# nirvanesque/headCT_foundation

Hardware: AMD Instinct MI355X
Metric: CT-volumes/sec MAE pretrain step (96^3, ViT-B/16^3, mask 0.75) (higher is better)
Workload: dtype bf16; 1 GPU; BASELINE config #2: MAE ViT-B/16^3, 96^3x1ch, mask 0.75, full train step (fwd+bwd+clip+AdamW+LR); per_gpu_batch=256, global_batch=256, parallelism=dp1, init=reference init, seed 42

## Files before the change

### headct_foundation_amd/_lib.py

```python
from __future__ import annotations

import ctypes as C
import os
from typing import Optional

HERE = os.path.dirname(os.path.abspath(__file__))
LIB_PATH = os.path.join(HERE, "libheadct_hip.so")

HCT_F32, HCT_BF16, HCT_F16 = 0, 1, 2
NORM_LAYERNORM, NORM_RMSNORM = 0, 1
HCT_ACT_NONE, HCT_ACT_GELU, HCT_ACT_DGELU, HCT_ACT_TANH, HCT_ACT_GELU_D, HCT_ACT_MULAUX = 0, 1, 2, 3, 4, 5
ACT_NONE, ACT_GELU, ACT_DGELU = 0, 1, 2

c_void_p, c_int, c_float, c_size_t, c_int64 = C.c_void_p, C.c_int, C.c_float, C.c_size_t, C.c_int64


class GemmArgs(C.Structure):
    _fields_ = [
        ("M", c_int), ("N", c_int), ("K", c_int),
        ("A", c_void_p), ("a_dtype", c_int), ("lda", c_int64), ("transA", c_int),
        ("B", c_void_p), ("b_dtype", c_int), ("ldb", c_int64), ("transB", c_int),
        ("C", c_void_p), ("c_dtype", c_int), ("ldc", c_int64),
        ("bias", c_void_p), ("residual", c_void_p), ("ldr", c_int64),
        ("act", c_int),
# ... 51 lines not shown
    "hct_assemble_bwd_workspace_bytes": (c_size_t, [c_int]),
    "hct_layernorm_fwd": (c_int, [c_void_p, c_void_p, c_void_p, c_int, c_int, c_float, c_void_p, c_int, c_void_p, c_void_p, c_void_p]),
    "hct_layernorm_bwd_workspace_bytes": (c_size_t, [c_int, c_int]),
    "hct_layernorm_bwd": (c_int, [c_void_p, c_int, c_void_p, c_void_p, c_void_p, c_void_p, c_void_p, c_int, c_int, c_void_p, c_void_p,
                                  c_int, c_void_p, c_void_p, c_void_p, c_void_p, c_size_t, c_void_p]),
    "hct_layernorm_bwd_mapped": (c_int, [c_void_p, c_int, c_void_p, c_void_p, c_void_p, c_void_p, c_void_p, c_void_p, c_int, c_int, c_void_p,
                                         c_void_p, c_int, c_void_p, c_void_p, c_void_p, c_void_p, c_size_t, c_void_p]),
    "hct_rmsnorm_fwd": (c_int, [c_void_p, c_void_p, c_int, c_int, c_float, c_void_p, c_int, c_void_p, c_void_p]),
    "hct_rmsnorm_bwd_workspace_bytes": (c_size_t, [c_int, c_int]),
    "hct_rmsnorm_bwd": (c_int, [c_void_p, c_int, c_void_p, c_void_p, c_void_p, c_void_p, c_int, c_int, c_void_p, c_void_p, c_int, c_void_p,
                                c_void_p, c_void_p, c_size_t, c_void_p]),
    "hct_rmsnorm_bwd_mapped": (c_int, [c_void_p, c_int, c_void_p, c_void_p, c_void_p, c_void_p, c_void_p, c_int, c_int, c_void_p, c_void_p,
                                       c_int, c_void_p, c_void_p, c_void_p, c_size_t, c_void_p]),
    "hct_tail_rows": (c_int, [c_void_p, c_int, c_int, c_int, c_void_p, c_void_p, c_void_p]),
    "hct_gather_rows": (c_int, [c_void_p, c_void_p, c_int, c_int, c_void_p, c_void_p]),
    "hct_attention_fwd": (c_int, [c_void_p, c_int, c_int, c_int, c_int, c_int, c_void_p, c_void_p, c_void_p]),
    "hct_attention_bwd": (c_int, [c_void_p, c_void_p, c_void_p, c_void_p, c_int, c_int, c_int, c_int, c_int, c_void_p, c_void_p]),
    "hct_debug_force_simple_attention": (None, [c_int]),
    "hct_decoder_assemble_fwd": (c_int, [c_void_p, c_int, c_void_p, c_void_p, c_void_p, c_void_p, c_int, c_int, c_int, c_int, c_void_p, c_void_p]),
    "hct_decoder_assemble_bwd": (c_int, [c_void_p, c_void_p, c_void_p, c_int, c_int, c_int, c_int, c_void_p, c_int, c_void_p, c_void_p,
                                         c_void_p, c_size_t, c_void_p]),
    "hct_masked_mse": (c_int, [c_void_p, c_int, c_void_p, c_int, c_void_p, c_int, c_int, c_int, c_int, c_int, c_float, c_void_p, c_void_p, c_void_p, c_void_p, c_void_p]),
    "hct_unpatchify": (c_int, [c_void_p, c_int, c_int, c_int, c_int, c_int, c_int, c_void_p, c_void_p]),
    "hct_vit_assemble_fwd": (c_int, [c_void_p, c_int, c_void_p, c_void_p, c_void_p, c_int, c_int, c_int, c_int, c_void_p, c_void_p]),
    "hct_channel_norm": (c_int, [c_void_p, c_void_p, c_void_p, c_float, c_void_p, c_int, c_int64, c_int, c_void_p]),
    "hct_query_attention": (c_int, [c_void_p, c_int, c_void_p, c_int, c_int, c_int, c_int, c_int, c_float, c_void_p, c_void_p]),
    "hct_head_linear": (c_int, [c_void_p, c_int64, c_int, c_void_p, c_void_p, c_float, c_void_p, c_void_p, c_int, c_void_p, c_int, c_int,
                                c_int, c_void_p]),
    "hct_batchnorm_stats": (c_int, [c_void_p, c_int, c_int, c_float, c_void_p, c_void_p, c_void_p, c_void_p, c_void_p]),
    "hct_softmax_xent": (c_int, [c_void_p, c_void_p, c_int, c_int, c_void_p, c_void_p, c_void_p, c_void_p]),
# ... 192 lines not shown
```

### headct_foundation_amd/csrc/common.h

```cpp
#pragma once
#include <hip/hip_runtime.h>
#include <stdint.h>
#include <stdio.h>
#include <string.h>

#include "../../include/headct_hip.h"

namespace hct {

typedef __bf16 bf16;
typedef _Float16 f16;
typedef __attribute__((ext_vector_type(4))) _Float16 f16x4;
typedef __attribute__((ext_vector_type(8))) __bf16 bf16x8;
typedef __attribute__((ext_vector_type(4))) __bf16 bf16x4;
typedef __attribute__((ext_vector_type(2))) __bf16 bf16x2;
typedef __attribute__((ext_vector_type(4))) short s16x4;
typedef __attribute__((ext_vector_type(4))) float f32x4;
typedef __attribute__((ext_vector_type(16))) float f32x16;

constexpr int kWave = 64;

void set_error(const char* fmt, ...);
int check_hip(hipError_t e, const char* what);
#define HCT_CHECK_LAUNCH(what)                         \
// ... 25 lines not shown
int fold_rows(const float* partial, int nblk, int D, float* out, hipStream_t s);

struct FoldJob {
  const float* partial;
  int nblk, nq_stride, D, nq;
  float* out[3];
};
struct FoldSink {
  static constexpr int kMax = 8;
  FoldJob jobs[kMax];
  int n = 0;
};
extern thread_local FoldSink* g_fold_sink;
int fold_partials(const FoldJob& job, hipStream_t s);
int fold_flush(FoldSink& sink, hipStream_t s);

inline size_t dtype_size(int dt) { return dt == HCT_BF16 ? 2 : 4; }
inline size_t align_up(size_t v, size_t a) { return (v + a - 1) / a * a; }

__device__ __forceinline__ float to_f32(float v) { return v; }
__device__ __forceinline__ float to_f32(bf16 v) { return (float)v; }
template <typename T> __device__ __forceinline__ T from_f32(float v);
template <> __device__ __forceinline__ float from_f32<float>(float v) { return v; }
template <> __device__ __forceinline__ bf16 from_f32<bf16>(float v) { return (bf16)v; }

template <typename T> struct Vec4;
template <> struct Vec4<float> {
  static __device__ __forceinline__ f32x4 load(const float* p) { return *reinterpret_cast<const f32x4*>(p); }
  static __device__ __forceinline__ void store(float* p, f32x4 v) { *reinterpret_cast<f32x4*>(p) = v; }
  static __device__ __forceinline__ f32x4 load_nt(const float* p) { return __builtin_nontemporal_load(reinterpret_cast<const f32x4*>(p)); }
// ... 119 lines not shown
```

### headct_foundation_amd/csrc/elementwise.hip

```cpp
#include "common.h"

#include <stdarg.h>
#include <algorithm>

namespace hct {

static thread_local char g_err[512] = "";
void set_error(const char* fmt, ...) {
  va_list ap;
  va_start(ap, fmt);
  vsnprintf(g_err, sizeof(g_err), fmt, ap);
  va_end(ap);
}
int check_hip(hipError_t e, const char* what) {
  if (e == hipSuccess) return 0;
  set_error("%s: %s", what, hipGetErrorString(e));
  return (int)e;
}

__global__ void mask_rank_kernel(const float* __restrict__ noise, int L, int K, int32_t* __restrict__ ids_restore,
                                 int32_t* __restrict__ ids_shuffle, float* __restrict__ mask) {
  extern __shared__ float s_noise[];
  const int b = blockIdx.x;
  const float* row = noise + (size_t)b * L;
  for (int i = threadIdx.x; i < L; i += blockDim.x) s_noise[i] = row[i];
  __syncthreads();
  for (int l = threadIdx.x; l < L; l += blockDim.x) {
    const float v = s_noise[l];
    int r = 0;
    for (int j = 0; j < L; ++j) {
      const float w = s_noise[j];
      r += (w < v) || (w == v && j < l);
// ... 73 lines not shown
    f32x4 v = Vec4<T>::load(src + d);
    if (pos) v += Vec4<float>::load(pos + (size_t)l * D + d);
    Vec4<float>::store(out + d, v);
  }
}

template <typename T>
__global__ void encoder_assemble_bwd_tok_kernel(const float* __restrict__ dh0, int K, int D, T* __restrict__ dtok) {
  const int r = blockIdx.x;
  const int b = r / K, j = r - b * K;
  const float* src = dh0 + ((size_t)b * (K + 1) + 1 + j) * D;
  T* out = dtok + (size_t)r * D;
  for (int d = threadIdx.x * 4; d < D; d += blockDim.x * 4) Vec4<T>::store(out + d, Vec4<float>::load(src + d));
}

__global__ void encoder_assemble_bwd_pos_kernel(const float* __restrict__ dh0, const int32_t* __restrict__ ids_restore,
                                                int B, int L, int K, int D, float* __restrict__ dpos) {
  const int l = blockIdx.x;
  for (int d = threadIdx.x * 4; d < D; d += blockDim.x * 4) {
    f32x4 acc = {0, 0, 0, 0};
    for (int b0 = 0; b0 < B; b0 += 8) {
      int r[8];
      f32x4 v[8];
#pragma unroll
      for (int u = 0; u < 8; ++u) r[u] = b0 + u < B ? ids_restore[(size_t)(b0 + u) * L + l] : K;
#pragma unroll
      for (int u = 0; u < 8; ++u)
        v[u] = r[u] < K ? Vec4<float>::load(dh0 + ((size_t)(b0 + u) * (K + 1) + 1 + r[u]) * D + d) : f32x4{0, 0, 0, 0};
#pragma unroll
      for (int u = 0; u < 8; ++u)
        if (r[u] < K) acc += v[u];
    }
    Vec4<float>::store(dpos + (size_t)l * D + d, acc);
  }
}

template <typename T>
__global__ void vit_assemble_bwd_tok_kernel(const float* __restrict__ dh0, int L, int R, int D, T* __restrict__ dtok) {
  const int r = blockIdx.x;
  const int b = r / L, l = r - b * L;
  const float* src = dh0 + ((size_t)b * (1 + R + L) + 1 + R + l) * D;
  T* out = dtok + (size_t)r * D;
  for (int d = threadIdx.x * 4; d < D; d += blockDim.x * 4) Vec4<T>::store(out + d, Vec4<float>::load(src + d));
}

__global__ void strided_rowsum_kernel(const float* __restrict__ src, int B, size_t stride, int D, float* __restrict__ out) {
  const int d = blockIdx.x * blockDim.x + threadIdx.x;
  if (d >= D) return;
  float acc = 0.f;
// ... 345 lines not shown
  }
}

template <typename T>
__global__ void decoder_assemble_bwd_kernel(const float* __restrict__ dy, const int32_t* __restrict__ ids_shuffle, int L,
                                            int K, int D, T* __restrict__ de) {
  const int r = blockIdx.x;
  const int b = r / (K + 1), t = r - b * (K + 1);
  const int srow = t == 0 ? 0 : 1 + ids_shuffle[(size_t)b * L + (t - 1)];
  const float* src = dy + ((size_t)b * (L + 1) + srow) * D;
  T* out = de + (size_t)r * D;
  for (int d = threadIdx.x * 4; d < D; d += blockDim.x * 4) Vec4<T>::store(out + d, Vec4<float>::load(src + d));
}

constexpr int kAsmBlocks = 256;
__global__ void decoder_assemble_bwd_reduce_kernel(const float* __restrict__ dy, const int32_t* __restrict__ ids_shuffle,
                                                   int B, int L, int K, int D, float* __restrict__ partial) {
  for (int d = threadIdx.x * 4; d < D; d += blockDim.x * 4) {
    f32x4 am = {0, 0, 0, 0}, ac = {0, 0, 0, 0};
    for (int b = blockIdx.x; b < B; b += gridDim.x) {
      const float* base = dy + (size_t)b * (L + 1) * D;
      ac += Vec4<float>::load(base + d);
      for (int j0 = K; j0 < L; j0 += 8) {
        int l[8];
        f32x4 v[8];
#pragma unroll
        for (int u = 0; u < 8; ++u) l[u] = j0 + u < L ? ids_shuffle[(size_t)b * L + j0 + u] : 0;
#pragma unroll
        for (int u = 0; u < 8; ++u) v[u] = Vec4<float>::load(base + (size_t)(1 + l[u]) * D + d);
#pragma unroll
        for (int u = 0; u < 8; ++u)
          if (j0 + u < L) am += v[u];
      }
    }
    Vec4<float>::store(partial + ((size_t)blockIdx.x * 2 + 0) * D + d, am);
    Vec4<float>::store(partial + ((size_t)blockIdx.x * 2 + 1) * D + d, ac);
  }
}

__device__ __forceinline__ float block_sum_256(float v, float* s_tmp) {
  v = wave_sum(v);
  __syncthreads();
  if ((threadIdx.x & 63) == 0) s_tmp[threadIdx.x >> 6] = v;
  __syncthreads();
  return (s_tmp[0] + s_tmp[1]) + (s_tmp[2] + s_tmp[3]);
}

template <typename TX, typename T>
__global__ void __launch_bounds__(256) masked_mse_kernel(const T* __restrict__ pred, const TX* __restrict__ x,
                                                         const float* __restrict__ mask, int C, int S, int P, int L,
                                                         int norm_pix, float inv_masksum, float* __restrict__ row_loss,
                                                         T* __restrict__ dpred, const float* __restrict__ dscale, float hscale,
// ... 486 lines not shown
  else {
    const int rank = ids_restore[(size_t)b * L + (t - 1)];
    c = rank < K ? b * (K + 1) + 1 + rank : Nc + (t - 1);
  }
  if (c < Nc) kept_rows[c] = r;
  cat_idx[r] = c;
}

__global__ void __launch_bounds__(256) dec0_table_kernel(const float* __restrict__ mask_token, const float* __restrict__ pos, int D,
                                                         float* __restrict__ out) {
  const int l = blockIdx.x;
  for (int d = threadIdx.x * 4; d < D; d += 1024)
    Vec4<float>::store(out + (size_t)l * D + d, Vec4<float>::load(mask_token + d) + Vec4<float>::load(pos + (size_t)l * D + d));
}

template <typename T>
__global__ void __launch_bounds__(256) dec0_table_sum_kernel(const T* __restrict__ g, const int32_t* __restrict__ ids_restore, int B, int L, int K,
                                                             int W, T* __restrict__ out) {
  __shared__ f32x4 s_part[4][64];
  const int l = blockIdx.x, q = threadIdx.x & 63, vg = threadIdx.x >> 6;
  const int col = blockIdx.y * 256 + q * 4;
  f32x4 acc = {0, 0, 0, 0};
  if (col < W) {
    for (int b0 = vg; b0 < B; b0 += 32) {
      int rk[8];
      f32x4 v[8];
#pragma unroll
      for (int u = 0; u < 8; ++u) rk[u] = b0 + 4 * u < B ? ids_restore[(size_t)(b0 + 4 * u) * L + l] : -1;
#pragma unroll
      for (int u = 0; u < 8; ++u)
        v[u] = rk[u] >= K ? Vec4<T>::load(g + ((size_t)(b0 + 4 * u) * (L + 1) + 1 + l) * W + col) : f32x4{0, 0, 0, 0};
#pragma unroll
      for (int u = 0; u < 8; ++u) acc += v[u];
    }
  }
  s_part[vg][q] = acc;
  __syncthreads();
  if (vg == 0 && col < W) Vec4<T>::store(out + (size_t)l * W + col, (s_part[0][q] + s_part[1][q]) + (s_part[2][q] + s_part[3][q]));
}

__global__ void __launch_bounds__(512) dec0_token_grads_kernel(const float* __restrict__ partial, int nblk, const float* __restrict__ dcat,
                                                               int B, int L, int K, int D, float* __restrict__ dmask, float* __restrict__ dcls) {
  __shared__ float s_m[16][32], s_c[16][32];
  const int c = threadIdx.x & 31, rg = threadIdx.x >> 5;
  const int d = blockIdx.x * 32 + c;
  const size_t Nc = (size_t)B * (K + 1);
  auto sum_rows = [&](const float* base, int n, size_t stride) {
    float acc = 0.f;
    for (int r0 = rg; r0 < n; r0 += 16 * 8) {
      float v[8];
#pragma unroll
      for (int u = 0; u < 8; ++u) v[u] = r0 + 16 * u < n ? base[(size_t)(r0 + 16 * u) * stride + d] : 0.f;
#pragma unroll
// ... 54 lines not shown
int dec0_index(const int32_t* ids_restore, int B, int L, int K, int32_t* kept_rows, int32_t* cat_idx, hipStream_t s) {
  const int n = std::max(B * (L + 1), L);
  hipLaunchKernelGGL(dec0_index_kernel, dim3((n + 255) / 256), dim3(256), 0, s, ids_restore, B, L, K, kept_rows, cat_idx);
  HCT_CHECK_LAUNCH("dec0_index");
  return 0;
}
int dec0_table(const float* mask_token, const float* pos, int L, int D, float* out, hipStream_t s) {
  hipLaunchKernelGGL(dec0_table_kernel, dim3(L), dim3(256), 0, s, mask_token, pos, D, out);
  HCT_CHECK_LAUNCH("dec0_table");
  return 0;
}
int dec0_aggregate(const void* g, int dtype, const int32_t* kept_rows, const int32_t* ids_restore, int B, int L, int K, int W, void* out, hipStream_t s) {
  HCT_REQUIRE(W % 4 == 0 && (W * dtype_size(dtype)) % 16 == 0, "dec0_aggregate: row width must be a multiple of 16 bytes");
  const int Nc = B * (K + 1);
  if (int rc = hct_gather_rows(g, kept_rows, Nc, (int)(W * dtype_size(dtype)), out, s)) return rc;
  const dim3 grid(L, (W + 255) / 256);
  HCT_DISPATCH_DTYPE(dtype, T, hipLaunchKernelGGL(dec0_table_sum_kernel<T>, grid, dim3(256), 0, s, (const T*)g, ids_restore, B, L, K, W, (T*)out + (size_t)Nc * W));
  HCT_CHECK_LAUNCH("dec0_aggregate");
  return 0;
}
int dec0_token_grads(const float* dh, const int32_t* ids_shuffle, const float* dcat, int B, int L, int K, int D, float* dmask, float* dcls,
                     void* workspace, size_t workspace_bytes, hipStream_t s) {
  if (workspace_bytes < hct_assemble_bwd_workspace_bytes(D)) {
    set_error("dec0_token_grads: workspace too small");
    return HCT_E_WORKSPACE;
  }
  const int threads = D / 4 >= 256 ? 256 : (D / 4 > 64 ? 128 : 64);
  const int nblk = std::min(B, kAsmBlocks);
  float* partial = (float*)workspace;
  hipLaunchKernelGGL(decoder_assemble_bwd_reduce_kernel, dim3(nblk), dim3(threads), 0, s, dh, ids_shuffle, B, L, K, D, partial);
  hipLaunchKernelGGL(dec0_token_grads_kernel, dim3((D + 31) / 32), dim3(512), 0, s, partial, nblk, dcat, B, L, K, D, dmask, dcls);
  HCT_CHECK_LAUNCH("dec0_token_grads");
  return 0;
}
}

extern "C" {

const char* hct_last_error_string(void) { return g_err; }
int hct_version(void) { return 100; }
int hct_has_mfma_kernels(void) { return 1; }

int hct_mask_rank(const float* noise, int B, int L, int K, int32_t* ids_restore, int32_t* ids_shuffle, float* mask,
                  void* stream) {
  HCT_REQUIRE(B > 0 && L > 0 && K >= 0 && K <= L && L <= 12288, "hct_mask_rank: bad shape B=%d L=%d K=%d", B, L, K);
// ... 48 lines not shown

size_t hct_assemble_bwd_workspace_bytes(int D) { return (size_t)kAsmBlocks * 2 * D * sizeof(float); }

int hct_encoder_assemble_bwd(const float* dh0, const int32_t* ids_restore, int B, int L, int K, int D, void* dtok,
                             int dtok_dtype, float* dcls, float* dpos, void* workspace, size_t workspace_bytes,
                             void* stream) {
  (void)workspace; (void)workspace_bytes;
  HCT_REQUIRE(D % 4 == 0, "hct_encoder_assemble_bwd: D %% 4 != 0 (%d)", D);
  const int threads = D / 4 >= 256 ? 256 : (D / 4 > 64 ? 128 : 64);
  hipStream_t s = (hipStream_t)stream;
  if (dtok && B * K > 0)
    HCT_DISPATCH_DTYPE(dtok_dtype, T,
                       hipLaunchKernelGGL(encoder_assemble_bwd_tok_kernel<T>, dim3(B * K), dim3(threads), 0, s, dh0, K, D,
                                          (T*)dtok));
  if (dcls) hipLaunchKernelGGL(strided_rowsum_kernel, dim3((D + 255) / 256), dim3(256), 0, s, dh0, B, (size_t)(K + 1) * D, D, dcls);
  if (dpos) hipLaunchKernelGGL(encoder_assemble_bwd_pos_kernel, dim3(L), dim3(threads), 0, s, dh0, ids_restore, B, L, K, D, dpos);
  HCT_CHECK_LAUNCH("hct_encoder_assemble_bwd");
  return 0;
}

int hct_vit_assemble_bwd(const float* dh0, int B, int L, int R, int D, void* dtok, int dtok_dtype, float* dcls, float* dreg, float* dpos,
                         void* stream) {
  HCT_REQUIRE(dh0 && B > 0 && L > 0 && R >= 0 && D > 0 && D % 4 == 0, "hct_vit_assemble_bwd: bad arguments");
  hipStream_t s = (hipStream_t)stream;
  const size_t stride = (size_t)(1 + R + L) * D;
  if (dtok) {
    HCT_DISPATCH_DTYPE(dtok_dtype, T, hipLaunchKernelGGL(hct::vit_assemble_bwd_tok_kernel<T>, dim3(B * L), dim3(D / 4 >= 256 ? 256 : 64), 0, s, dh0, L,
                                                        R, D, (T*)dtok));
  }
  if (dcls) hipLaunchKernelGGL(strided_rowsum_kernel, dim3((D + 255) / 256), dim3(256), 0, s, dh0, B, stride, D, dcls);
  if (dreg && R > 0) hipLaunchKernelGGL(strided_rowsum_kernel, dim3((R * D + 255) / 256), dim3(256), 0, s, dh0 + D, B, stride, R * D, dreg);
  if (dpos) hipLaunchKernelGGL(strided_rowsum_kernel, dim3((L * D + 255) / 256), dim3(256), 0, s, dh0 + (size_t)(1 + R) * D, B, stride, L * D, dpos);
  HCT_CHECK_LAUNCH("hct_vit_assemble_bwd");
  return 0;
}

int hct_layernorm_fwd(const float* x, const float* gamma, const float* beta, int rows, int D, float eps, void* y,
                      int y_dtype, float* mean, float* rstd, void* stream) {
  HCT_REQUIRE(D % 4 == 0 && rows >= 0, "hct_layernorm_fwd: bad shape rows=%d D=%d", rows, D);
  if (rows == 0) return 0;
  const int nblk = min((rows + 3) / 4, 2048);
#define HCT_LN_FWD(NV_)                                                                                                 \
  HCT_DISPATCH_DTYPE(y_dtype, T,                                                                                       \
                     hipLaunchKernelGGL((layernorm_fwd_reg_kernel<T, NV_>), dim3(nblk), dim3(256), 0, (hipStream_t)stream, x, \
                                        gamma, beta, rows, D, eps, (T*)y, mean, rstd))
  if (D <= 256) HCT_LN_FWD(1);
  else if (D <= 512) HCT_LN_FWD(2);
  else if (D <= 768) HCT_LN_FWD(3);
  else if (D <= 1024) HCT_LN_FWD(4);
  else
    HCT_DISPATCH_DTYPE(y_dtype, T,
                       hipLaunchKernelGGL(layernorm_fwd_kernel<T>, dim3((rows + 3) / 4), dim3(256), 0, (hipStream_t)stream,
                                          x, gamma, beta, rows, D, eps, (T*)y, mean, rstd));
#undef HCT_LN_FWD
  HCT_CHECK_LAUNCH("hct_layernorm_fwd");
  return 0;
}

size_t hct_layernorm_bwd_workspace_bytes(int rows, int D) {
  (void)rows;
// ... 26 lines not shown
    if (dx_shadow && shadow_dtype == HCT_F32) rc = launch_ln_bwd<bf16, float>(dy, x, mean, rstd, gamma, dres, dres_rows, rows, D, dx, dx_shadow, partial, dcolsum != nullptr, nblk, s);
    else rc = launch_ln_bwd<bf16, bf16>(dy, x, mean, rstd, gamma, dres, dres_rows, rows, D, dx, dx_shadow, partial, dcolsum != nullptr, nblk, s);
  } else {
    if (dx_shadow && shadow_dtype == HCT_BF16) rc = launch_ln_bwd<float, bf16>(dy, x, mean, rstd, gamma, dres, dres_rows, rows, D, dx, dx_shadow, partial, dcolsum != nullptr, nblk, s);
    else rc = launch_ln_bwd<float, float>(dy, x, mean, rstd, gamma, dres, dres_rows, rows, D, dx, dx_shadow, partial, dcolsum != nullptr, nblk, s);
  }
  if (rc) return rc;
  HCT_CHECK_LAUNCH("hct_layernorm_bwd");
  return fold_partials(FoldJob{partial, nblk, 3, D, dcolsum ? 3 : 2, {dgamma, dbeta, dcolsum}}, s);
}

int hct_rmsnorm_fwd(const float* x, const float* gamma, int rows, int D, float eps, void* y, int y_dtype, float* rstd,
                    void* stream) {
  HCT_REQUIRE(D % 4 == 0 && rows >= 0, "hct_rmsnorm_fwd: bad shape rows=%d D=%d", rows, D);
  if (rows == 0) return 0;
  const int nblk = min((rows + 3) / 4, 2048);
#define HCT_RMS_FWD(NV_)                                                                                                     \
  HCT_DISPATCH_DTYPE(y_dtype, T,                                                                                             \
                     hipLaunchKernelGGL((rmsnorm_fwd_reg_kernel<T, NV_>), dim3(nblk), dim3(256), 0, (hipStream_t)stream, x, gamma, \
                                        rows, D, eps, (T*)y, rstd))
  if (D <= 256) HCT_RMS_FWD(1);
  else if (D <= 512) HCT_RMS_FWD(2);
  else if (D <= 768) HCT_RMS_FWD(3);
  else if (D <= 1024) HCT_RMS_FWD(4);
  else
    HCT_DISPATCH_DTYPE(y_dtype, T,
                       hipLaunchKernelGGL(rmsnorm_fwd_kernel<T>, dim3((rows + 3) / 4), dim3(256), 0, (hipStream_t)stream, x, gamma,
                                          rows, D, eps, (T*)y, rstd));
#undef HCT_RMS_FWD
  HCT_CHECK_LAUNCH("hct_rmsnorm_fwd");
  return 0;
}

size_t hct_rmsnorm_bwd_workspace_bytes(int rows, int D) { return hct_layernorm_bwd_workspace_bytes(rows, D); }

// ... 47 lines not shown
                             int K, int D, void* de, int de_dtype, float* dmask_token, float* ddec_cls,
                             void* workspace, size_t workspace_bytes, void* stream) {
  (void)ids_restore;
  HCT_REQUIRE(D % 4 == 0, "hct_decoder_assemble_bwd: D %% 4 != 0 (%d)", D);
  if (workspace_bytes < hct_assemble_bwd_workspace_bytes(D)) {
    set_error("hct_decoder_assemble_bwd: workspace too small");
    return HCT_E_WORKSPACE;
  }
  hipStream_t s = (hipStream_t)stream;
  const int threads = D / 4 >= 256 ? 256 : (D / 4 > 64 ? 128 : 64);
  HCT_DISPATCH_DTYPE(de_dtype, T,
                     hipLaunchKernelGGL(decoder_assemble_bwd_kernel<T>, dim3(B * (K + 1)), dim3(threads), 0, s, dy,
                                        ids_shuffle, L, K, D, (T*)de));
  const int nblk = min(B, kAsmBlocks);
  float* partial = (float*)workspace;
  hipLaunchKernelGGL(decoder_assemble_bwd_reduce_kernel, dim3(nblk), dim3(threads), 0, s, dy, ids_shuffle, B, L, K, D, partial);
  hipLaunchKernelGGL(fold_partials_kernel, dim3((D + 31) / 32, 2), dim3(kFoldThreads), 0, s, partial, nblk, 2, D, dmask_token,
                     ddec_cls, (float*)nullptr);
  HCT_CHECK_LAUNCH("hct_decoder_assemble_bwd");
  return 0;
}

int hct_masked_mse(const void* pred, int pred_dtype, const void* x, int x_dtype, const float* mask, int B, int C, int S, int P,
                   int norm_pix, float mask_sum, float* row_loss, float* loss, void* dpred, const float* dpred_scale,
                   void* stream) {
  return masked_mse_launch(pred, pred_dtype, x, x_dtype, mask, B, C, S, P, norm_pix, mask_sum, row_loss, loss, dpred, dpred_scale, 1.0f,
                           (hipStream_t)stream, nullptr, 0);
}

int hct_tail_rows(const int32_t* ids_restore, int B, int L, int K, int32_t* tail_rows, int32_t* tail_inv, void* stream) {
  HCT_REQUIRE(ids_restore && tail_rows && tail_inv && B > 0 && L > 0 && K >= 0 && K < L, "hct_tail_rows: bad arguments");
  const int n = B * (L + 1);
  hipLaunchKernelGGL(hct::tail_rows_kernel, dim3((n + 255) / 256), dim3(256), 0, (hipStream_t)stream, ids_restore, B, L, K, tail_rows, tail_inv);
  HCT_CHECK_LAUNCH("hct_tail_rows");
  return 0;
}

int hct_gather_rows(const void* src, const int32_t* idx, int n_rows, int row_bytes, void* dst, void* stream) {
  HCT_REQUIRE(src && idx && dst && n_rows >= 0 && row_bytes > 0 && row_bytes % 16 == 0 && ((uintptr_t)src % 16) == 0 && ((uintptr_t)dst % 16) == 0,
              "hct_gather_rows: bad arguments (rows of a multiple of 16 bytes, 16-byte aligned)");
  if (n_rows == 0) return 0;
  const int64_t total = (int64_t)n_rows * (row_bytes / 16);
// ... 145 lines not shown
```

### headct_foundation_amd/csrc/mae_plan.hip

```cpp
#include <cstdlib>
#include "common.h"

#include <algorithm>
#include <map>
#include <string>
#include <vector>

using namespace hct;

namespace {

constexpr int64_t kUnitElems = 1024;

struct BlockP {
  int ln1_w, ln1_b, qkv_w, qkv_b, proj_w, proj_b, ln2_w, ln2_b, fc1_w, fc1_b, fc2_w, fc2_b;
  int lq_b = -1, lq_a = -1, lv_b = -1, lv_a = -1;
};
struct BlockA {
  size_t x1, mean1, rstd1, qkv, o, lse, h_mid, x2, mean2, rstd2, u, g;
  size_t lora_t = 0;
};
struct Act { size_t off; int64_t rows, cols; int dtype; };
struct BlockG { size_t out, big, mid, qkv, lora_du = 0, lora_dt = 0; };
constexpr int kWgSlots = 8;
// ... 107 lines not shown
  b.fc1_w = add_param(p, pre + ".mlp.linear1.weight", {m, d}, true, true, true);
  b.fc1_b = add_param(p, pre + ".mlp.linear1.bias", {m}, true, false, false);
  b.fc2_w = add_param(p, pre + ".mlp.linear2.weight", {d, m}, true, true, true);
  b.fc2_b = add_param(p, pre + ".mlp.linear2.bias", {d}, true, false, false);
  return b;
}

constexpr int kMaxT = 112;
struct TransposeTable {
  int n;
  int tile_start[kMaxT + 1];
  int rows[kMaxT], cols[kMaxT];
  long long src[kMaxT], dst[kMaxT];
};

__global__ void __launch_bounds__(256) transpose_cast_batched_kernel(const float* __restrict__ src, bf16* __restrict__ dst,
                                                                     TransposeTable t) {
  __shared__ float tile[64][65];
  int lo = 0, hi = t.n;
  while (hi - lo > 1) {
    const int mid = (lo + hi) >> 1;
    if (t.tile_start[mid] <= (int)blockIdx.x) lo = mid; else hi = mid;
  }
  const int rows = t.rows[lo], cols = t.cols[lo];
  const int local = blockIdx.x - t.tile_start[lo];
  const int tcols = (cols + 63) >> 6;
  const int r0 = (local / tcols) * 64, c0 = (local % tcols) * 64;
  const float* s = src + t.src[lo];
  bf16* d = dst + t.dst[lo];
  const int q = threadIdx.x & 15, rr = threadIdx.x >> 4;
  const bool vec = (cols & 3) == 0 && (rows & 3) == 0;
  if (vec) {
#pragma unroll
    for (int i = 0; i < 4; ++i) {
      const int r = r0 + rr + 16 * i, c = c0 + q * 4;
      f32x4 v = {0, 0, 0, 0};
      if (r < rows && c < cols) v = Vec4<float>::load(s + (size_t)r * cols + c);
#pragma unroll
      for (int e = 0; e < 4; ++e) tile[rr + 16 * i][q * 4 + e] = v[e];
    }
    __syncthreads();
#pragma unroll
    for (int i = 0; i < 4; ++i) {
      const int c = c0 + rr + 16 * i, r = r0 + q * 4;
      if (c < cols && r < rows) {
        const f32x4 v = {tile[q * 4 + 0][rr + 16 * i], tile[q * 4 + 1][rr + 16 * i], tile[q * 4 + 2][rr + 16 * i], tile[q * 4 + 3][rr + 16 * i]};
        Vec4<bf16>::store(d + (size_t)c * rows + r, v);
      }
    }
    return;
  }
  const int tx = threadIdx.x & 63, ty = threadIdx.x >> 6;
  for (int i = ty; i < 64; i += 4) {
    const int r = r0 + i, c = c0 + tx;
    tile[i][tx] = (r < rows && c < cols) ? s[(size_t)r * cols + c] : 0.f;
  }
  __syncthreads();
  for (int i = ty; i < 64; i += 4) {
    const int c = c0 + i, r = r0 + tx;
    if (c < cols && r < rows) d[(size_t)c * rows + r] = (bf16)tile[tx][i];
  }
}

struct WsAlloc {
  size_t cur = 0;
  size_t take(size_t bytes) {
    size_t o = cur;
    cur += align_up(bytes ? bytes : 16, 256);
    return o;
  }
// ... 645 lines not shown
  p->fwd_done = false;
  for (auto& v : p->wg_prepared) v.clear();
  p->wg_pending.clear();
  return 0;
}

int hct_mae_refresh_weights(hct_mae_plan* p, int with_plain, void* stream) {
  HCT_REQUIRE(p && p->params_f32, "hct_mae_refresh_weights: plan not bound");
  if (p->dt != HCT_BF16) return 0;
  if (with_plain) RC(hct_cast(p->params_f32, HCT_F32, p->params_bf16, HCT_BF16, p->param_elems, stream));
  TransposeTable t;
  t.n = 0;
  t.tile_start[0] = 0;
  auto flush = [&]() -> int {
    if (t.n == 0) return 0;
    hipLaunchKernelGGL(transpose_cast_batched_kernel, dim3(t.tile_start[t.n]), dim3(256), 0, (hipStream_t)stream, p->params_f32,
                       p->params_bf16_t, t);
    t.n = 0;
    return check_hip(hipGetLastError(), "hct_mae_refresh_weights");
  };
  for (const auto& pi : p->params) {
    if (pi.bf16_t_offset < 0) continue;
    if (!with_plain && p->t_all_done && !pi.requires_grad) continue;
    const int rows = (int)pi.shape[0], cols = (int)(pi.numel / pi.shape[0]);
    t.rows[t.n] = rows; t.cols[t.n] = cols; t.src[t.n] = pi.offset; t.dst[t.n] = pi.bf16_t_offset;
    t.tile_start[t.n + 1] = t.tile_start[t.n] + ((rows + 63) / 64) * ((cols + 63) / 64);
    if (++t.n == kMaxT) RC(flush());
  }
  RC(flush());
  p->t_all_done = true;
  return 0;
// ... 220 lines not shown
```

### include/headct_hip.h

```cpp
#ifndef HEADCT_HIP_H
#define HEADCT_HIP_H

#include <stddef.h>
#include <stdint.h>

#ifdef __cplusplus
extern "C" {
#endif

#define HCT_F32 0
#define HCT_BF16 1
#define HCT_F16 2

#define HCT_E_BADARG (-1)
#define HCT_E_UNSUPPORTED (-2)
#define HCT_E_WORKSPACE (-3)
#define HCT_E_STATE (-4)

#define HCT_ACT_NONE 0
#define HCT_ACT_GELU 1
#define HCT_ACT_DGELU 2
#define HCT_ACT_TANH 3
#define HCT_ACT_GELU_D 4
#define HCT_ACT_MULAUX 5
// ... 51 lines not shown
int hct_layernorm_bwd_mapped(const void* dy, int dy_dtype, const float* x, const float* mean, const float* rstd,
                             const float* gamma, const float* dres, const int32_t* dres_rows, int rows, int D, float* dx,
                             void* dx_shadow, int shadow_dtype, float* dgamma, float* dbeta, float* dcolsum, void* workspace,
                             size_t workspace_bytes, void* stream);
int hct_rmsnorm_fwd(const float* x, const float* gamma, int rows, int D, float eps, void* y, int y_dtype, float* rstd,
                    void* stream);
size_t hct_rmsnorm_bwd_workspace_bytes(int rows, int D);
int hct_rmsnorm_bwd(const void* dy, int dy_dtype, const float* x, const float* rstd, const float* gamma, const float* dres,
                    int rows, int D, float* dx, void* dx_shadow, int shadow_dtype, float* dgamma, float* dcolsum,
                    void* workspace, size_t workspace_bytes, void* stream);
int hct_rmsnorm_bwd_mapped(const void* dy, int dy_dtype, const float* x, const float* rstd, const float* gamma,
                           const float* dres, const int32_t* dres_rows, int rows, int D, float* dx, void* dx_shadow,
                           int shadow_dtype, float* dgamma, float* dcolsum, void* workspace, size_t workspace_bytes,
                           void* stream);
int hct_tail_rows(const int32_t* ids_restore, int B, int L, int K, int32_t* tail_rows, int32_t* tail_inv, void* stream);
int hct_gather_rows(const void* src, const int32_t* idx, int n_rows, int row_bytes, void* dst, void* stream);

int hct_attention_fwd(const void* qkv, int B, int N, int H, int dh, int dtype, void* o, float* lse, void* stream);
int hct_attention_bwd(const void* qkv, const void* o, const void* d_o, const float* lse, int B, int N, int H,
                      int dh, int dtype, void* dqkv, void* stream);

int hct_decoder_assemble_fwd(const void* e, int e_dtype, const float* mask_token, const float* dec_cls,
                             const float* dec_pos, const int32_t* ids_restore, int B, int L, int K, int D,
                             float* y, void* stream);
int hct_decoder_assemble_bwd(const float* dy, const int32_t* ids_restore, const int32_t* ids_shuffle, int B,
                             int L, int K, int D, void* de, int de_dtype, float* dmask_token, float* ddec_cls,
                             void* workspace, size_t workspace_bytes, void* stream);

int hct_masked_mse(const void* pred, int pred_dtype, const void* x, int x_dtype , const float* mask, int B, int C, int S,
                   int P, int norm_pix, float mask_sum, float* row_loss, float* loss, void* dpred,
// ... 199 lines not shown
```

Measured before the change: 6934 CT-volumes/s.

## Retune gather-reduce kernels, size norm grids by occupancy, transpose from bf16 weights

Several memory-bound kernels are reworked. The encoder positional-gradient and decoder assemble reduction kernels now use 64-thread blocks with a second grid dimension over columns, and prefetch the next batch of indices. The decoder table-sum kernel loads 16 bytes per lane for bf16 and is exposed as a public entry point. LayerNorm and RMSNorm forward grids are capped by occupancy-derived resident block counts rather than a fixed 2048. The weight-refresh transpose now reads the bf16 parameter copy instead of fp32, which assumes that copy is already current when refresh runs.

```diff
diff --git a/headct_foundation_amd/_lib.py b/headct_foundation_amd/_lib.py
--- a/headct_foundation_amd/_lib.py
+++ b/headct_foundation_amd/_lib.py
@@ -89,6 +89,7 @@
                                        c_int, c_void_p, c_void_p, c_void_p, c_size_t, c_void_p]),
     "hct_tail_rows": (c_int, [c_void_p, c_int, c_int, c_int, c_void_p, c_void_p, c_void_p]),
     "hct_gather_rows": (c_int, [c_void_p, c_void_p, c_int, c_int, c_void_p, c_void_p]),
+    "hct_dec0_table_sum": (c_int, [c_void_p, c_int, c_void_p, c_int, c_int, c_int, c_int, c_void_p, c_void_p]),
     "hct_attention_fwd": (c_int, [c_void_p, c_int, c_int, c_int, c_int, c_int, c_void_p, c_void_p, c_void_p]),
     "hct_attention_bwd": (c_int, [c_void_p, c_void_p, c_void_p, c_void_p, c_int, c_int, c_int, c_int, c_int, c_void_p, c_void_p]),
     "hct_debug_force_simple_attention": (None, [c_int]),
diff --git a/headct_foundation_amd/csrc/common.h b/headct_foundation_amd/csrc/common.h
--- a/headct_foundation_amd/csrc/common.h
+++ b/headct_foundation_amd/csrc/common.h
@@ -63,6 +63,16 @@
 extern thread_local FoldSink* g_fold_sink;
 int fold_partials(const FoldJob& job, hipStream_t s);
 int fold_flush(FoldSink& sink, hipStream_t s);
+
+int device_cus();
+template <typename K> inline int resident_blocks(K kernel, int threads, int fallback) {
+  int per_cu = 0;
+  if (hipOccupancyMaxActiveBlocksPerMultiprocessor(&per_cu, kernel, threads, 0) != hipSuccess || per_cu <= 0) {
+    (void)hipGetLastError();
+    return fallback;
+  }
+  return per_cu * device_cus();
+}
 
 inline size_t dtype_size(int dt) { return dt == HCT_BF16 ? 2 : 4; }
 inline size_t align_up(size_t v, size_t a) { return (v + a - 1) / a * a; }
diff --git a/headct_foundation_amd/csrc/elementwise.hip b/headct_foundation_amd/csrc/elementwise.hip
--- a/headct_foundation_amd/csrc/elementwise.hip
+++ b/headct_foundation_amd/csrc/elementwise.hip
@@ -16,6 +16,15 @@
   if (e == hipSuccess) return 0;
   set_error("%s: %s", what, hipGetErrorString(e));
   return (int)e;
+}
+int device_cus() {
+  static const int n = [] {
+    int dev = 0;
+    hipDeviceProp_t prop;
+    const bool ok = hipGetDevice(&dev) == hipSuccess && hipGetDeviceProperties(&prop, dev) == hipSuccess && prop.multiProcessorCount > 0;
+    return ok ? prop.multiProcessorCount : 256;
+  }();
+  return n;
 }
 
 __global__ void mask_rank_kernel(const float* __restrict__ noise, int L, int K, int32_t* __restrict__ ids_restore,
@@ -119,25 +128,33 @@
   for (int d = threadIdx.x * 4; d < D; d += blockDim.x * 4) Vec4<T>::store(out + d, Vec4<float>::load(src + d));
 }
 
-__global__ void encoder_assemble_bwd_pos_kernel(const float* __restrict__ dh0, const int32_t* __restrict__ ids_restore,
-                                                int B, int L, int K, int D, float* __restrict__ dpos) {
-  const int l = blockIdx.x;
-  for (int d = threadIdx.x * 4; d < D; d += blockDim.x * 4) {
-    f32x4 acc = {0, 0, 0, 0};
-    for (int b0 = 0; b0 < B; b0 += 8) {
-      int r[8];
-      f32x4 v[8];
-#pragma unroll
-      for (int u = 0; u < 8; ++u) r[u] = b0 + u < B ? ids_restore[(size_t)(b0 + u) * L + l] : K;
-#pragma unroll
-      for (int u = 0; u < 8; ++u)
-        v[u] = r[u] < K ? Vec4<float>::load(dh0 + ((size_t)(b0 + u) * (K + 1) + 1 + r[u]) * D + d) : f32x4{0, 0, 0, 0};
-#pragma unroll
-      for (int u = 0; u < 8; ++u)
+constexpr int kPosBatch = 32;
+__global__ void __launch_bounds__(64) encoder_assemble_bwd_pos_kernel(const float* __restrict__ dh0, const int32_t* __restrict__ ids_restore,
+                                                                      int B, int L, int K, int D, float* __restrict__ dpos) {
+  const int l = blockIdx.x, lane = threadIdx.x;
+  const int d = blockIdx.y * 256 + lane * 4;
+  const bool act = d < D;
+  f32x4 acc = {0, 0, 0, 0};
+  int mine = lane < B ? ids_restore[(size_t)lane * L + l] : K;
+  for (int c0 = 0; c0 < B; c0 += 64) {
+    const int nb = c0 + 64 + lane;
+    const int next = nb < B ? ids_restore[(size_t)nb * L + l] : K;
+#pragma unroll
+    for (int h = 0; h < 64; h += kPosBatch) {
+      int r[kPosBatch];
+      f32x4 v[kPosBatch];
+#pragma unroll
+      for (int u = 0; u < kPosBatch; ++u) r[u] = __builtin_amdgcn_readlane(mine, h + u);
+#pragma unroll
+      for (int u = 0; u < kPosBatch; ++u)
+        v[u] = (r[u] < K && act) ? Vec4<float>::load(dh0 + ((size_t)(c0 + h + u) * (K + 1) + 1 + r[u]) * D + d) : f32x4{0, 0, 0, 0};
+#pragma unroll
+      for (int u = 0; u < kPosBatch; ++u)
         if (r[u] < K) acc += v[u];
     }
-    Vec4<float>::store(dpos + (size_t)l * D + d, acc);
-  }
+    mine = next;
+  }
+  if (act) Vec4<float>::store(dpos + (size_t)l * D + d, acc);
 }
 
 template <typename T>
@@ -513,28 +530,33 @@
 }
 
 constexpr int kAsmBlocks = 256;
-__global__ void decoder_assemble_bwd_reduce_kernel(const float* __restrict__ dy, const int32_t* __restrict__ ids_shuffle,
-                                                   int B, int L, int K, int D, float* __restrict__ partial) {
-  for (int d = threadIdx.x * 4; d < D; d += blockDim.x * 4) {
-    f32x4 am = {0, 0, 0, 0}, ac = {0, 0, 0, 0};
-    for (int b = blockIdx.x; b < B; b += gridDim.x) {
-      const float* base = dy + (size_t)b * (L + 1) * D;
-      ac += Vec4<float>::load(base + d);
-      for (int j0 = K; j0 < L; j0 += 8) {
-        int l[8];
-        f32x4 v[8];
-#pragma unroll
-        for (int u = 0; u < 8; ++u) l[u] = j0 + u < L ? ids_shuffle[(size_t)b * L + j0 + u] : 0;
-#pragma unroll
-        for (int u = 0; u < 8; ++u) v[u] = Vec4<float>::load(base + (size_t)(1 + l[u]) * D + d);
-#pragma unroll
-        for (int u = 0; u < 8; ++u)
-          if (j0 + u < L) am += v[u];
-      }
-    }
-    Vec4<float>::store(partial + ((size_t)blockIdx.x * 2 + 0) * D + d, am);
-    Vec4<float>::store(partial + ((size_t)blockIdx.x * 2 + 1) * D + d, ac);
-  }
+constexpr int kAsmBatch = 16;
+__global__ void __launch_bounds__(64) decoder_assemble_bwd_reduce_kernel(const float* __restrict__ dy, const int32_t* __restrict__ ids_shuffle,
+                                                                         int B, int L, int K, int D, float* __restrict__ partial) {
+  const int d = blockIdx.y * 256 + threadIdx.x * 4;
+  if (d >= D) return;
+  f32x4 am = {0, 0, 0, 0}, ac = {0, 0, 0, 0};
+  for (int b = blockIdx.x; b < B; b += gridDim.x) {
+    const float* base = dy + (size_t)b * (L + 1) * D;
+    ac += Vec4<float>::load(base + d);
+    int l[kAsmBatch], ln[kAsmBatch];
+#pragma unroll
+    for (int u = 0; u < kAsmBatch; ++u) l[u] = K + u < L ? ids_shuffle[(size_t)b * L + K + u] : 0;
+    for (int j0 = K; j0 < L; j0 += kAsmBatch) {
+      f32x4 v[kAsmBatch];
+#pragma unroll
+      for (int u = 0; u < kAsmBatch; ++u) v[u] = Vec4<float>::load(base + (size_t)(1 + l[u]) * D + d);
+#pragma unroll
+      for (int u = 0; u < kAsmBatch; ++u) ln[u] = j0 + kAsmBatch + u < L ? ids_shuffle[(size_t)b * L + j0 + kAsmBatch + u] : 0;
+#pragma unroll
+      for (int u = 0; u < kAsmBatch; ++u)
+        if (j0 + u < L) am += v[u];
+#pragma unroll
+      for (int u = 0; u < kAsmBatch; ++u) l[u] = ln[u];
+    }
+  }
+  Vec4<float>::store(partial + ((size_t)blockIdx.x * 2 + 0) * D + d, am);
+  Vec4<float>::store(partial + ((size_t)blockIdx.x * 2 + 1) * D + d, ac);
 }
 
 __device__ __forceinline__ float block_sum_256(float v, float* s_tmp) {
@@ -1051,29 +1073,51 @@
     Vec4<float>::store(out + (size_t)l * D + d, Vec4<float>::load(mask_token + d) + Vec4<float>::load(pos + (size_t)l * D + d));
 }
 
-template <typename T>
+constexpr int kTabBatch = 8;
+template <typename T, int NQ>
 __global__ void __launch_bounds__(256) dec0_table_sum_kernel(const T* __restrict__ g, const int32_t* __restrict__ ids_restore, int B, int L, int K,
                                                              int W, T* __restrict__ out) {
-  __shared__ f32x4 s_part[4][64];
+  static_assert(NQ == 1 || (NQ == 2 && sizeof(T) == 2), "a lane loads 16 bytes");
+  typedef __attribute__((ext_vector_type(4 * NQ))) T RawVec;
+  __shared__ f32x4 s_part[4][NQ][64];
   const int l = blockIdx.x, q = threadIdx.x & 63, vg = threadIdx.x >> 6;
-  const int col = blockIdx.y * 256 + q * 4;
-  f32x4 acc = {0, 0, 0, 0};
+  const int col = (blockIdx.y * 64 + q) * (4 * NQ);
+  f32x4 acc[NQ];
+#pragma unroll
+  for (int h = 0; h < NQ; ++h) acc[h] = f32x4{0, 0, 0, 0};
   if (col < W) {
-    for (int b0 = vg; b0 < B; b0 += 32) {
-      int rk[8];
-      f32x4 v[8];
-#pragma unroll
-      for (int u = 0; u < 8; ++u) rk[u] = b0 + 4 * u < B ? ids_restore[(size_t)(b0 + 4 * u) * L + l] : -1;
-#pragma unroll
-      for (int u = 0; u < 8; ++u)
-        v[u] = rk[u] >= K ? Vec4<T>::load(g + ((size_t)(b0 + 4 * u) * (L + 1) + 1 + l) * W + col) : f32x4{0, 0, 0, 0};
-#pragma unroll
-      for (int u = 0; u < 8; ++u) acc += v[u];
-    }
-  }
-  s_part[vg][q] = acc;
+    int rk[kTabBatch], rn[kTabBatch];
+#pragma unroll
+    for (int u = 0; u < kTabBatch; ++u) rk[u] = vg + 4 * u < B ? ids_restore[(size_t)(vg + 4 * u) * L + l] : -1;
+    for (int b0 = vg; b0 < B; b0 += 4 * kTabBatch) {
+      RawVec v[kTabBatch];
+#pragma unroll
+      for (int u = 0; u < kTabBatch; ++u) {
+        if (rk[u] >= K) v[u] = *reinterpret_cast<const RawVec*>(g + ((size_t)(b0 + 4 * u) * (L + 1) + 1 + l) * W + col);
+        else v[u] = RawVec(0);
+      }
+#pragma unroll
+      for (int u = 0; u < kTabBatch; ++u) {
+        const int bn = b0 + 4 * (kTabBatch + u);
+        rn[u] = bn < B ? ids_restore[(size_t)bn * L + l] : -1;
+      }
+#pragma unroll
+      for (int u = 0; u < kTabBatch; ++u)
+#pragma unroll
+        for (int h = 0; h < NQ; ++h)
+          acc[h] += f32x4{to_f32(v[u][4 * h]), to_f32(v[u][4 * h + 1]), to_f32(v[u][4 * h + 2]), to_f32(v[u][4 * h + 3])};
+#pragma unroll
+      for (int u = 0; u < kTabBatch; ++u) rk[u] = rn[u];
+    }
+  }
+#pragma unroll
+  for (int h = 0; h < NQ; ++h) s_part[vg][h][q] = acc[h];
   __syncthreads();
-  if (vg == 0 && col < W) Vec4<T>::store(out + (size_t)l * W + col, (s_part[0][q] + s_part[1][q]) + (s_part[2][q] + s_part[3][q]));
+  if (vg == 0 && col < W) {
+#pragma unroll
+    for (int h = 0; h < NQ; ++h)
+      Vec4<T>::store(out + (size_t)l * W + col + 4 * h, (s_part[0][h][q] + s_part[1][h][q]) + (s_part[2][h][q] + s_part[3][h][q]));
+  }
 }
 
 __global__ void __launch_bounds__(512) dec0_token_grads_kernel(const float* __restrict__ partial, int nblk, const float* __restrict__ dcat,
@@ -1158,8 +1202,7 @@
   HCT_REQUIRE(W % 4 == 0 && (W * dtype_size(dtype)) % 16 == 0, "dec0_aggregate: row width must be a multiple of 16 bytes");
   const int Nc = B * (K + 1);
   if (int rc = hct_gather_rows(g, kept_rows, Nc, (int)(W * dtype_size(dtype)), out, s)) return rc;
-  const dim3 grid(L, (W + 255) / 256);
-  HCT_DISPATCH_DTYPE(dtype, T, hipLaunchKernelGGL(dec0_table_sum_kernel<T>, grid, dim3(256), 0, s, (const T*)g, ids_restore, B, L, K, W, (T*)out + (size_t)Nc * W));
+  if (int rc = hct_dec0_table_sum(g, dtype, ids_restore, B, L, K, W, (char*)out + (size_t)Nc * W * dtype_size(dtype), s)) return rc;
   HCT_CHECK_LAUNCH("dec0_aggregate");
   return 0;
 }
@@ -1169,10 +1212,9 @@
     set_error("dec0_token_grads: workspace too small");
     return HCT_E_WORKSPACE;
   }
-  const int threads = D / 4 >= 256 ? 256 : (D / 4 > 64 ? 128 : 64);
   const int nblk = std::min(B, kAsmBlocks);
   float* partial = (float*)workspace;
-  hipLaunchKernelGGL(decoder_assemble_bwd_reduce_kernel, dim3(nblk), dim3(threads), 0, s, dh, ids_shuffle, B, L, K, D, partial);
+  hipLaunchKernelGGL(decoder_assemble_bwd_reduce_kernel, dim3(nblk, (D + 255) / 256), dim3(64), 0, s, dh, ids_shuffle, B, L, K, D, partial);
   hipLaunchKernelGGL(dec0_token_grads_kernel, dim3((D + 31) / 32), dim3(512), 0, s, partial, nblk, dcat, B, L, K, D, dmask, dcls);
   HCT_CHECK_LAUNCH("dec0_token_grads");
   return 0;
@@ -1251,7 +1293,7 @@
                        hipLaunchKernelGGL(encoder_assemble_bwd_tok_kernel<T>, dim3(B * K), dim3(threads), 0, s, dh0, K, D,
                                           (T*)dtok));
   if (dcls) hipLaunchKernelGGL(strided_rowsum_kernel, dim3((D + 255) / 256), dim3(256), 0, s, dh0, B, (size_t)(K + 1) * D, D, dcls);
-  if (dpos) hipLaunchKernelGGL(encoder_assemble_bwd_pos_kernel, dim3(L), dim3(threads), 0, s, dh0, ids_restore, B, L, K, D, dpos);
+  if (dpos) hipLaunchKernelGGL(encoder_assemble_bwd_pos_kernel, dim3(L, (D + 255) / 256), dim3(64), 0, s, dh0, ids_restore, B, L, K, D, dpos);
   HCT_CHECK_LAUNCH("hct_encoder_assemble_bwd");
   return 0;
 }
@@ -1276,11 +1318,12 @@
                       int y_dtype, float* mean, float* rstd, void* stream) {
   HCT_REQUIRE(D % 4 == 0 && rows >= 0, "hct_layernorm_fwd: bad shape rows=%d D=%d", rows, D);
   if (rows == 0) return 0;
-  const int nblk = min((rows + 3) / 4, 2048);
 #define HCT_LN_FWD(NV_)                                                                                                 \
-  HCT_DISPATCH_DTYPE(y_dtype, T,                                                                                       \
-                     hipLaunchKernelGGL((layernorm_fwd_reg_kernel<T, NV_>), dim3(nblk), dim3(256), 0, (hipStream_t)stream, x, \
-                                        gamma, beta, rows, D, eps, (T*)y, mean, rstd))
+  HCT_DISPATCH_DTYPE(y_dtype, T, {                                                                                     \
+    static const int resident = resident_blocks(layernorm_fwd_reg_kernel<T, NV_>, 256, 2048);               \
+    hipLaunchKernelGGL((layernorm_fwd_reg_kernel<T, NV_>), dim3(min((rows + 3) / 4, resident)), dim3(256), 0, \
+                       (hipStream_t)stream, x, gamma, beta, rows, D, eps, (T*)y, mean, rstd);                           \
+  })
   if (D <= 256) HCT_LN_FWD(1);
   else if (D <= 512) HCT_LN_FWD(2);
   else if (D <= 768) HCT_LN_FWD(3);
@@ -1337,11 +1380,12 @@
                     void* stream) {
   HCT_REQUIRE(D % 4 == 0 && rows >= 0, "hct_rmsnorm_fwd: bad shape rows=%d D=%d", rows, D);
   if (rows == 0) return 0;
-  const int nblk = min((rows + 3) / 4, 2048);
-#define HCT_RMS_FWD(NV_)                                                                                                     \
-  HCT_DISPATCH_DTYPE(y_dtype, T,                                                                                             \
-                     hipLaunchKernelGGL((rmsnorm_fwd_reg_kernel<T, NV_>), dim3(nblk), dim3(256), 0, (hipStream_t)stream, x, gamma, \
-                                        rows, D, eps, (T*)y, rstd))
+#define HCT_RMS_FWD(NV_)                                                                  \
+  HCT_DISPATCH_DTYPE(y_dtype, T, {                                                                                      \
+    static const int resident = resident_blocks(rmsnorm_fwd_reg_kernel<T, NV_>, 256, 2048);                             \
+    hipLaunchKernelGGL((rmsnorm_fwd_reg_kernel<T, NV_>), dim3(min((rows + 3) / 4, resident)), dim3(256), 0,             \
+                       (hipStream_t)stream, x, gamma, rows, D, eps, (T*)y, rstd);                                       \
+  })
   if (D <= 256) HCT_RMS_FWD(1);
   else if (D <= 512) HCT_RMS_FWD(2);
   else if (D <= 768) HCT_RMS_FWD(3);
@@ -1419,7 +1463,7 @@
                                         ids_shuffle, L, K, D, (T*)de));
   const int nblk = min(B, kAsmBlocks);
   float* partial = (float*)workspace;
-  hipLaunchKernelGGL(decoder_assemble_bwd_reduce_kernel, dim3(nblk), dim3(threads), 0, s, dy, ids_shuffle, B, L, K, D, partial);
+  hipLaunchKernelGGL(decoder_assemble_bwd_reduce_kernel, dim3(nblk, (D + 255) / 256), dim3(64), 0, s, dy, ids_shuffle, B, L, K, D, partial);
   hipLaunchKernelGGL(fold_partials_kernel, dim3((D + 31) / 32, 2), dim3(kFoldThreads), 0, s, partial, nblk, 2, D, dmask_token,
                      ddec_cls, (float*)nullptr);
   HCT_CHECK_LAUNCH("hct_decoder_assemble_bwd");
@@ -1431,6 +1475,20 @@
                    void* stream) {
   return masked_mse_launch(pred, pred_dtype, x, x_dtype, mask, B, C, S, P, norm_pix, mask_sum, row_loss, loss, dpred, dpred_scale, 1.0f,
                            (hipStream_t)stream, nullptr, 0);
+}
+
+int hct_dec0_table_sum(const void* g, int dtype, const int32_t* ids_restore, int B, int L, int K, int W, void* out, void* stream) {
+  HCT_REQUIRE(g && ids_restore && out && B > 0 && L > 0 && K >= 0 && W > 0, "hct_dec0_table_sum: bad arguments");
+  HCT_REQUIRE(W % 4 == 0, "hct_dec0_table_sum: row width must be a multiple of 4 elements (%d)", W);
+  hipStream_t s = (hipStream_t)stream;
+  if (dtype == HCT_BF16 && W % 8 == 0)
+    hipLaunchKernelGGL((dec0_table_sum_kernel<bf16, 2>), dim3(L, (W + 511) / 512), dim3(256), 0, s, (const bf16*)g, ids_restore, B, L, K, W,
+                       (bf16*)out);
+  else
+    HCT_DISPATCH_DTYPE(dtype, T, hipLaunchKernelGGL((dec0_table_sum_kernel<T, 1>), dim3(L, (W + 255) / 256), dim3(256), 0, s, (const T*)g,
+                                                    ids_restore, B, L, K, W, (T*)out));
+  HCT_CHECK_LAUNCH("hct_dec0_table_sum");
+  return 0;
 }
 
 int hct_tail_rows(const int32_t* ids_restore, int B, int L, int K, int32_t* tail_rows, int32_t* tail_inv, void* stream) {
diff --git a/headct_foundation_amd/csrc/mae_plan.hip b/headct_foundation_amd/csrc/mae_plan.hip
--- a/headct_foundation_amd/csrc/mae_plan.hip
+++ b/headct_foundation_amd/csrc/mae_plan.hip
@@ -145,8 +145,7 @@
   long long src[kMaxT], dst[kMaxT];
 };
 
-__global__ void __launch_bounds__(256) transpose_cast_batched_kernel(const float* __restrict__ src, bf16* __restrict__ dst,
-                                                                     TransposeTable t) {
+__global__ void __launch_bounds__(256) transpose_bf16_batched_kernel(const bf16* __restrict__ src, bf16* __restrict__ dst, TransposeTable t) {
   __shared__ float tile[64][65];
   int lo = 0, hi = t.n;
   while (hi - lo > 1) {
@@ -157,8 +156,31 @@
   const int local = blockIdx.x - t.tile_start[lo];
   const int tcols = (cols + 63) >> 6;
   const int r0 = (local / tcols) * 64, c0 = (local % tcols) * 64;
-  const float* s = src + t.src[lo];
+  const bf16* s = src + t.src[lo];
   bf16* d = dst + t.dst[lo];
+  if ((cols & 7) == 0 && (rows & 7) == 0) {
+    const int q = threadIdx.x & 7, rr = threadIdx.x >> 3;
+#pragma unroll
+    for (int i = 0; i < 2; ++i) {
+      const int r = r0 + rr + 32 * i, c = c0 + q * 8;
+      bf16x8 v = {0, 0, 0, 0, 0, 0, 0, 0};
+      if (r < rows && c < cols) v = *reinterpret_cast<const bf16x8*>(s + (size_t)r * cols + c);
+#pragma unroll
+      for (int e = 0; e < 8; ++e) tile[rr + 32 * i][q * 8 + e] = (float)v[e];
+    }
+    __syncthreads();
+#pragma unroll
+    for (int i = 0; i < 2; ++i) {
+      const int c = c0 + rr + 32 * i, r = r0 + q * 8;
+      if (c < cols && r < rows) {
+        bf16x8 v;
+#pragma unroll
+        for (int e = 0; e < 8; ++e) v[e] = (bf16)tile[q * 8 + e][rr + 32 * i];
+        *reinterpret_cast<bf16x8*>(d + (size_t)c * rows + r) = v;
+      }
+    }
+    return;
+  }
   const int q = threadIdx.x & 15, rr = threadIdx.x >> 4;
   const bool vec = (cols & 3) == 0 && (rows & 3) == 0;
   if (vec) {
@@ -166,7 +188,7 @@
     for (int i = 0; i < 4; ++i) {
       const int r = r0 + rr + 16 * i, c = c0 + q * 4;
       f32x4 v = {0, 0, 0, 0};
-      if (r < rows && c < cols) v = Vec4<float>::load(s + (size_t)r * cols + c);
+      if (r < rows && c < cols) v = Vec4<bf16>::load(s + (size_t)r * cols + c);
 #pragma unroll
       for (int e = 0; e < 4; ++e) tile[rr + 16 * i][q * 4 + e] = v[e];
     }
@@ -184,7 +206,7 @@
   const int tx = threadIdx.x & 63, ty = threadIdx.x >> 6;
   for (int i = ty; i < 64; i += 4) {
     const int r = r0 + i, c = c0 + tx;
-    tile[i][tx] = (r < rows && c < cols) ? s[(size_t)r * cols + c] : 0.f;
+    tile[i][tx] = (r < rows && c < cols) ? (float)s[(size_t)r * cols + c] : 0.f;
   }
   __syncthreads();
   for (int i = ty; i < 64; i += 4) {
@@ -860,7 +882,7 @@
   t.tile_start[0] = 0;
   auto flush = [&]() -> int {
     if (t.n == 0) return 0;
-    hipLaunchKernelGGL(transpose_cast_batched_kernel, dim3(t.tile_start[t.n]), dim3(256), 0, (hipStream_t)stream, p->params_f32,
+    hipLaunchKernelGGL(transpose_bf16_batched_kernel, dim3(t.tile_start[t.n]), dim3(256), 0, (hipStream_t)stream, p->params_bf16,
                        p->params_bf16_t, t);
     t.n = 0;
     return check_hip(hipGetLastError(), "hct_mae_refresh_weights");
diff --git a/include/headct_hip.h b/include/headct_hip.h
--- a/include/headct_hip.h
+++ b/include/headct_hip.h
@@ -89,6 +89,7 @@
                            int shadow_dtype, float* dgamma, float* dcolsum, void* workspace, size_t workspace_bytes,
                            void* stream);
 int hct_tail_rows(const int32_t* ids_restore, int B, int L, int K, int32_t* tail_rows, int32_t* tail_inv, void* stream);
+int hct_dec0_table_sum(const void* g, int dtype, const int32_t* ids_restore, int B, int L, int K, int W, void* out, void* stream);
 int hct_gather_rows(const void* src, const int32_t* idx, int n_rows, int row_bytes, void* dst, void* stream);
 
 int hct_attention_fwd(const void* qkv, int B, int N, int H, int dh, int dtype, void* o, float* lse, void* stream);
```

Result: no change. 6962 CT-volumes/s (median of 6 runs) (+0.4%).
